# setarehc/diffusion-motion-inbetweening

Measured on NVIDIA H100. Metric: denoising steps/sec (B=64, L=196, D=263, 1000 steps), higher is better.
Workload: dtype bf16x3 (bf16 hi/lo operand split, fp32 accumulate: fp32-parity mode)

## Files before the change

diffusion-motion-inbetweening_b200/csrc/attention.cu:

```cuda
#include "common.cuh"
#include "gemm_epilogue.cuh"
#include "kernels.h"

namespace cmdi {

namespace {

constexpr int kHeadDim = 128;
constexpr int kQTile = 128;
constexpr int kKeyPad = kAttnKeyPad;
constexpr int kKeyBlocks = kKeyPad / 16;
constexpr int kQBlockBytes = kQTile * 128;
constexpr int kKVBlockBytes = kKeyPad * 128;
constexpr int kQPlane = 2 * kQBlockBytes;
constexpr int kKVPlane = 2 * kKVBlockBytes;
constexpr int kOffQHi = 0, kOffQLo = kQPlane;
constexpr int kOffKHi = 2 * kQPlane, kOffKLo = kOffKHi + kKVPlane;
constexpr int kOffVHi = kOffKLo + kKVPlane;
constexpr int kOffVLo = 0;
constexpr int kSmemTiles = kOffVHi + kKVPlane;
constexpr int kThreads = 256;
static_assert(kKVBlockBytes % 1024 == 0 && kKVPlane <= 2 * kQPlane, "operand tile layout");

struct __align__(8) AttnBarriers {
  uint64_t qkv_full, vlo_full;
};

__global__ void __launch_bounds__(kThreads, 1)
attention_kernel(const __grid_constant__ CUtensorMap map_q_hi, const __grid_constant__ CUtensorMap map_q_lo,
                 const __grid_constant__ CUtensorMap map_kv_hi, const __grid_constant__ CUtensorMap map_kv_lo, const AttnParams p) {
  extern __shared__ uint8_t smem_raw[];
  uint8_t* smem = reinterpret_cast<uint8_t*>((reinterpret_cast<uintptr_t>(smem_raw) + 1023) & ~uintptr_t(1023));
  AttnBarriers* bars = reinterpret_cast<AttnBarriers*>(smem + kSmemTiles);
  const int S = p.seq_len;
  const bool split = (p.nsplit == 3);
  const int half = blockIdx.x & 1;
  const int item = blockIdx.x >> 1;
  const int head = item % p.num_heads, seq = item / p.num_heads;
  if (half * kQTile >= S) return;
  const int warp_idx = threadIdx.x >> 5, lane = threadIdx.x & 31;
  const int wg = warp_idx >> 2, w = warp_idx & 3;
  const uint32_t sbase = smem_u32(smem);
  const int row0 = seq * S;
  const int kcol = p.num_heads * kHeadDim + head * kHeadDim, vcol = 2 * p.num_heads * kHeadDim + head * kHeadDim;
  const uint32_t planes = split ? 2 : 1;

  if (threadIdx.x == 0) {
    tma_prefetch_desc(&map_q_hi);
    tma_prefetch_desc(&map_kv_hi);
    mbar_init(&bars->qkv_full, 1);
    mbar_init(&bars->vlo_full, 1);
    fence_barrier_init();
    mbar_arrive_expect_tx(&bars->qkv_full, planes * (kQPlane + kKVPlane) + kKVPlane);
    for (int j = 0; j < 2; ++j) {
      tma_load_2d(smem + kOffQHi + j * kQBlockBytes, &map_q_hi, &bars->qkv_full, head * kHeadDim + j * 64, row0 + half * kQTile);
      tma_load_2d(smem + kOffKHi + j * kKVBlockBytes, &map_kv_hi, &bars->qkv_full, kcol + j * 64, row0);
      tma_load_2d(smem + kOffVHi + j * kKVBlockBytes, &map_kv_hi, &bars->qkv_full, vcol + j * 64, row0);
      if (split) {
        tma_load_2d(smem + kOffQLo + j * kQBlockBytes, &map_q_lo, &bars->qkv_full, head * kHeadDim + j * 64, row0 + half * kQTile);
        tma_load_2d(smem + kOffKLo + j * kKVBlockBytes, &map_kv_lo, &bars->qkv_full, kcol + j * 64, row0);
      }
    }
  }
  __syncthreads();

  float s[kKeyPad / 2];
  mbar_wait(&bars->qkv_full, 0);
  wgmma_fence_operands(s);
  wgmma_fence();
  {
    const int nterms = split ? 3 : 1;
#pragma unroll
    for (int term = 0; term < 3; ++term) {
      if (term >= nterms) break;
      const uint32_t qo = (split && term == 0) ? kOffQLo : kOffQHi;
      const uint32_t ko = (split && term == 1) ? kOffKLo : kOffKHi;
#pragma unroll
      for (int j = 0; j < 2; ++j) {
        const uint64_t da = make_desc_kmajor_sw128(sbase + qo + j * kQBlockBytes + wg * 64 * 128);
        const uint64_t db = make_desc_kmajor_sw128(sbase + ko + j * kKVBlockBytes);
#pragma unroll
        for (int kk = 0; kk < 4; ++kk)
          wgmma_m64n208k16_ss(s, desc_advance(da, kk * 32), desc_advance(db, kk * 32), (term | j | kk) ? 1u : 0u);
      }
    }
  }
  wgmma_commit();
  wgmma_wait<0>();
  wgmma_fence_operands(s);
  __syncthreads();
  if (split && threadIdx.x == 0) {
    mbar_arrive_expect_tx(&bars->vlo_full, kKVPlane);
    for (int j = 0; j < 2; ++j)
      tma_load_2d(smem + kOffVLo + j * kKVBlockBytes, &map_kv_lo, &bars->vlo_full, vcol + j * 64, row0);
  }

  const float c_scale = 0.08838834764831845f * 1.4426950408889634f;
  const int cq = 2 * (lane & 3);
  float mx0 = -INFINITY, mx1 = -INFINITY;
#pragma unroll
  for (int j = 0; j < kKeyPad / 8; ++j) {
    const bool ok0 = 8 * j + cq < S, ok1 = 8 * j + cq + 1 < S;
    if (!ok0) { s[4 * j] = -INFINITY; s[4 * j + 2] = -INFINITY; }
    if (!ok1) { s[4 * j + 1] = -INFINITY; s[4 * j + 3] = -INFINITY; }
    mx0 = fmaxf(mx0, fmaxf(s[4 * j], s[4 * j + 1]));
    mx1 = fmaxf(mx1, fmaxf(s[4 * j + 2], s[4 * j + 3]));
  }
#pragma unroll
  for (int o = 1; o <= 2; o <<= 1) {
    mx0 = fmaxf(mx0, __shfl_xor_sync(0xffffffffu, mx0, o));
    mx1 = fmaxf(mx1, __shfl_xor_sync(0xffffffffu, mx1, o));
  }
  const float mc0 = mx0 * c_scale, mc1 = mx1 * c_scale;
  float sum0 = 0.f, sum1 = 0.f;
  const bool trunc = p.trunc_split != 0;
  uint32_t ph[kKeyBlocks][4], pl[kKeyBlocks][4];
#pragma unroll
  for (int t = 0; t < kKeyBlocks; ++t) {
#pragma unroll
    for (int q = 0; q < 4; ++q) {
      const int i = 8 * t + 4 * (q >> 1) + 2 * (q & 1);
      const float mc = (q & 1) ? mc1 : mc0;
      const float p0 = fast_exp2(fmaf(s[i], c_scale, -mc));
      const float p1 = fast_exp2(fmaf(s[i + 1], c_scale, -mc));
      if (q & 1) sum1 += p0 + p1; else sum0 += p0 + p1;
      if (trunc) split_bf16x2_trunc(p0, p1, ph[t][q], pl[t][q]); else split_bf16x2(p0, p1, ph[t][q], pl[t][q]);
    }
  }
#pragma unroll
  for (int o = 1; o <= 2; o <<= 1) {
    sum0 += __shfl_xor_sync(0xffffffffu, sum0, o);
    sum1 += __shfl_xor_sync(0xffffffffu, sum1, o);
  }

  float o[kHeadDim / 2];
  const uint64_t dv_hi = make_desc_mnmajor_sw128(sbase + kOffVHi, kKVBlockBytes);
  wgmma_fence_operands(o);
  wgmma_fence();
  if (split) {
#pragma unroll
    for (int t = 0; t < kKeyBlocks; ++t) wgmma_m64n128k16_rs_tb(o, pl[t], desc_advance(dv_hi, t * 2048), t ? 1u : 0u);
  }
#pragma unroll
  for (int t = 0; t < kKeyBlocks; ++t) wgmma_m64n128k16_rs_tb(o, ph[t], desc_advance(dv_hi, t * 2048), (split || t) ? 1u : 0u);
  wgmma_commit();
  if (split) {
    mbar_wait(&bars->vlo_full, 0);
    const uint64_t dv_lo = make_desc_mnmajor_sw128(sbase + kOffVLo, kKVBlockBytes);
#pragma unroll
    for (int t = 0; t < kKeyBlocks; ++t) wgmma_m64n128k16_rs_tb(o, ph[t], desc_advance(dv_lo, t * 2048), 1u);
    wgmma_commit();
  }
  wgmma_wait<0>();
  wgmma_fence_operands(o);

  const float inv0 = 1.0f / sum0, inv1 = 1.0f / sum1;
  const int q0 = half * kQTile + wg * 64 + 16 * w + (lane >> 2);
#pragma unroll
  for (int g = 0; g < 2; ++g) {
    const int q = q0 + 8 * g;
    if (q >= S) continue;
    const float inv = g ? inv1 : inv0;
    const size_t off = (size_t)(row0 + q) * p.ld_out + head * kHeadDim + cq;
#pragma unroll
    for (int j = 0; j < kHeadDim / 8; ++j) {
      uint32_t hw, lw;
      if (trunc) split_bf16x2_trunc(o[4 * j + 2 * g] * inv, o[4 * j + 2 * g + 1] * inv, hw, lw);
      else split_bf16x2(o[4 * j + 2 * g] * inv, o[4 * j + 2 * g + 1] * inv, hw, lw);
      *reinterpret_cast<uint32_t*>(p.out_hi + off + 8 * j) = hw;
      if (p.nsplit_out == 3) *reinterpret_cast<uint32_t*>(p.out_lo + off + 8 * j) = lw;
    }
  }
}

}

cudaError_t configure_attention_kernel() {
  return cudaFuncSetAttribute(attention_kernel, cudaFuncAttributeMaxDynamicSharedMemorySize,
                              (int)(1024 + kSmemTiles + sizeof(AttnBarriers)));
}

cudaError_t launch_attention(const AttnMaps& m, const AttnParams& p, cudaStream_t stream) {
  if (p.seq_len > kKeyPad || p.seq_len < 1 || (p.nsplit != 1 && p.nsplit != 3)) {
    set_last_error("launch_attention: unsupported seq_len=%d nsplit=%d", p.seq_len, p.nsplit);
    return cudaErrorInvalidValue;
  }
  const int num_items = p.num_heads * p.num_seqs;
  const size_t smem = 1024 + kSmemTiles + sizeof(AttnBarriers);
  return launch_kernel(attention_kernel, dim3(2 * num_items), dim3(kThreads), smem, stream, *m.q_hi, *m.q_lo, *m.kv_hi, *m.kv_lo, p);
}

}
```

Before: 208.2.

## Make attention kernel persistent with per-operand barriers and next-item TMA prefetch

Converts the one-block-per-(seq,head,half) attention kernel into a persistent kernel with one block per SM looping over work items. Q, K-hi, K-lo, V-hi and V-lo get separate mbarriers with phase tracking, so the next item's operands can be loaded by TMA while the current item's softmax and PV run. V-lo now reuses the K-lo region instead of the Q region, which lets Q be prefetched early. The aim is to hide load latency and per-block launch/setup cost. The trade-offs are extra syncthreads, a cudaGetDevice/attribute query on every launch, and serialised item processing within each SM, since only one block fits per SM.

Result: no change. 210.0, median of 6 (+0.9%).

```diff
diff --git a/diffusion-motion-inbetweening_b200/csrc/attention.cu b/diffusion-motion-inbetweening_b200/csrc/attention.cu
--- a/diffusion-motion-inbetweening_b200/csrc/attention.cu
+++ b/diffusion-motion-inbetweening_b200/csrc/attention.cu
@@ -15,16 +15,46 @@
 constexpr int kQPlane = 2 * kQBlockBytes;
 constexpr int kKVPlane = 2 * kKVBlockBytes;
 constexpr int kOffQHi = 0, kOffQLo = kQPlane;
-constexpr int kOffKHi = 2 * kQPlane, kOffKLo = kOffKHi + kKVPlane;
+constexpr int kOffKHi = 2 * kQPlane;
+constexpr int kOffKLo = kOffKHi + kKVPlane, kOffVLo = kOffKLo;
 constexpr int kOffVHi = kOffKLo + kKVPlane;
-constexpr int kOffVLo = 0;
 constexpr int kSmemTiles = kOffVHi + kKVPlane;
 constexpr int kThreads = 256;
-static_assert(kKVBlockBytes % 1024 == 0 && kKVPlane <= 2 * kQPlane, "operand tile layout");
+static_assert(kKVBlockBytes % 1024 == 0, "operand tile layout");
 
 struct __align__(8) AttnBarriers {
-  uint64_t qkv_full, vlo_full;
+  uint64_t q_full, khi_full, klo_full, vhi_full, vlo_full;
 };
+
+struct AttnItem {
+  int row0, qrow, kcol, vcol, head;
+};
+
+__device__ __forceinline__ AttnItem attn_item(int it, int nhalves, const AttnParams& p) {
+  const int half = it % nhalves, hs = it / nhalves;
+  const int head = hs % p.num_heads, seq = hs / p.num_heads;
+  AttnItem r;
+  r.row0 = seq * p.seq_len;
+  r.qrow = r.row0 + half * kQTile;
+  r.head = head;
+  r.kcol = p.num_heads * kHeadDim + head * kHeadDim;
+  r.vcol = 2 * p.num_heads * kHeadDim + head * kHeadDim;
+  return r;
+}
+
+__device__ __forceinline__ void load_kv_plane(uint8_t* dst, const CUtensorMap* map, uint64_t* bar, int col, int row0) {
+  mbar_arrive_expect_tx(bar, kKVPlane);
+  for (int j = 0; j < 2; ++j) tma_load_2d(dst + j * kKVBlockBytes, map, bar, col + j * 64, row0);
+}
+
+__device__ __forceinline__ void load_q(uint8_t* smem, const CUtensorMap* map_hi, const CUtensorMap* map_lo, uint64_t* bar,
+                                       const AttnItem& t, bool split) {
+  mbar_arrive_expect_tx(bar, (split ? 2 : 1) * kQPlane);
+  for (int j = 0; j < 2; ++j) {
+    tma_load_2d(smem + kOffQHi + j * kQBlockBytes, map_hi, bar, t.head * kHeadDim + j * 64, t.qrow);
+    if (split) tma_load_2d(smem + kOffQLo + j * kQBlockBytes, map_lo, bar, t.head * kHeadDim + j * 64, t.qrow);
+  }
+}
 
 __global__ void __launch_bounds__(kThreads, 1)
 attention_kernel(const __grid_constant__ CUtensorMap map_q_hi, const __grid_constant__ CUtensorMap map_q_lo,
@@ -34,141 +64,153 @@
   AttnBarriers* bars = reinterpret_cast<AttnBarriers*>(smem + kSmemTiles);
   const int S = p.seq_len;
   const bool split = (p.nsplit == 3);
-  const int half = blockIdx.x & 1;
-  const int item = blockIdx.x >> 1;
-  const int head = item % p.num_heads, seq = item / p.num_heads;
-  if (half * kQTile >= S) return;
+  const int nhalves = (S + kQTile - 1) / kQTile;
+  const int num_items = nhalves * p.num_heads * p.num_seqs;
   const int warp_idx = threadIdx.x >> 5, lane = threadIdx.x & 31;
   const int wg = warp_idx >> 2, w = warp_idx & 3;
   const uint32_t sbase = smem_u32(smem);
-  const int row0 = seq * S;
-  const int kcol = p.num_heads * kHeadDim + head * kHeadDim, vcol = 2 * p.num_heads * kHeadDim + head * kHeadDim;
-  const uint32_t planes = split ? 2 : 1;
-
-  if (threadIdx.x == 0) {
+  const bool trunc = p.trunc_split != 0;
+  const int cq = 2 * (lane & 3);
+
+  if (threadIdx.x == 0 && (int)blockIdx.x < num_items) {
     tma_prefetch_desc(&map_q_hi);
     tma_prefetch_desc(&map_kv_hi);
-    mbar_init(&bars->qkv_full, 1);
+    mbar_init(&bars->q_full, 1);
+    mbar_init(&bars->khi_full, 1);
+    mbar_init(&bars->klo_full, 1);
+    mbar_init(&bars->vhi_full, 1);
     mbar_init(&bars->vlo_full, 1);
     fence_barrier_init();
-    mbar_arrive_expect_tx(&bars->qkv_full, planes * (kQPlane + kKVPlane) + kKVPlane);
-    for (int j = 0; j < 2; ++j) {
-      tma_load_2d(smem + kOffQHi + j * kQBlockBytes, &map_q_hi, &bars->qkv_full, head * kHeadDim + j * 64, row0 + half * kQTile);
-      tma_load_2d(smem + kOffKHi + j * kKVBlockBytes, &map_kv_hi, &bars->qkv_full, kcol + j * 64, row0);
-      tma_load_2d(smem + kOffVHi + j * kKVBlockBytes, &map_kv_hi, &bars->qkv_full, vcol + j * 64, row0);
-      if (split) {
-        tma_load_2d(smem + kOffQLo + j * kQBlockBytes, &map_q_lo, &bars->qkv_full, head * kHeadDim + j * 64, row0 + half * kQTile);
-        tma_load_2d(smem + kOffKLo + j * kKVBlockBytes, &map_kv_lo, &bars->qkv_full, kcol + j * 64, row0);
-      }
-    }
+    const AttnItem t = attn_item(blockIdx.x, nhalves, p);
+    load_q(smem, &map_q_hi, &map_q_lo, &bars->q_full, t, split);
+    load_kv_plane(smem + kOffKHi, &map_kv_hi, &bars->khi_full, t.kcol, t.row0);
+    if (split) load_kv_plane(smem + kOffKLo, &map_kv_lo, &bars->klo_full, t.kcol, t.row0);
+    load_kv_plane(smem + kOffVHi, &map_kv_hi, &bars->vhi_full, t.vcol, t.row0);
   }
   __syncthreads();
 
-  float s[kKeyPad / 2];
-  mbar_wait(&bars->qkv_full, 0);
-  wgmma_fence_operands(s);
-  wgmma_fence();
-  {
-    const int nterms = split ? 3 : 1;
-#pragma unroll
-    for (int term = 0; term < 3; ++term) {
-      if (term >= nterms) break;
-      const uint32_t qo = (split && term == 0) ? kOffQLo : kOffQHi;
-      const uint32_t ko = (split && term == 1) ? kOffKLo : kOffKHi;
-#pragma unroll
-      for (int j = 0; j < 2; ++j) {
-        const uint64_t da = make_desc_kmajor_sw128(sbase + qo + j * kQBlockBytes + wg * 64 * 128);
-        const uint64_t db = make_desc_kmajor_sw128(sbase + ko + j * kKVBlockBytes);
-#pragma unroll
-        for (int kk = 0; kk < 4; ++kk)
-          wgmma_m64n208k16_ss(s, desc_advance(da, kk * 32), desc_advance(db, kk * 32), (term | j | kk) ? 1u : 0u);
-      }
-    }
-  }
-  wgmma_commit();
-  wgmma_wait<0>();
-  wgmma_fence_operands(s);
-  __syncthreads();
-  if (split && threadIdx.x == 0) {
-    mbar_arrive_expect_tx(&bars->vlo_full, kKVPlane);
-    for (int j = 0; j < 2; ++j)
-      tma_load_2d(smem + kOffVLo + j * kKVBlockBytes, &map_kv_lo, &bars->vlo_full, vcol + j * 64, row0);
-  }
-
-  const float c_scale = 0.08838834764831845f * 1.4426950408889634f;
-  const int cq = 2 * (lane & 3);
-  float mx0 = -INFINITY, mx1 = -INFINITY;
-#pragma unroll
-  for (int j = 0; j < kKeyPad / 8; ++j) {
-    const bool ok0 = 8 * j + cq < S, ok1 = 8 * j + cq + 1 < S;
-    if (!ok0) { s[4 * j] = -INFINITY; s[4 * j + 2] = -INFINITY; }
-    if (!ok1) { s[4 * j + 1] = -INFINITY; s[4 * j + 3] = -INFINITY; }
-    mx0 = fmaxf(mx0, fmaxf(s[4 * j], s[4 * j + 1]));
-    mx1 = fmaxf(mx1, fmaxf(s[4 * j + 2], s[4 * j + 3]));
-  }
-#pragma unroll
-  for (int o = 1; o <= 2; o <<= 1) {
-    mx0 = fmaxf(mx0, __shfl_xor_sync(0xffffffffu, mx0, o));
-    mx1 = fmaxf(mx1, __shfl_xor_sync(0xffffffffu, mx1, o));
-  }
-  const float mc0 = mx0 * c_scale, mc1 = mx1 * c_scale;
-  float sum0 = 0.f, sum1 = 0.f;
-  const bool trunc = p.trunc_split != 0;
-  uint32_t ph[kKeyBlocks][4], pl[kKeyBlocks][4];
-#pragma unroll
-  for (int t = 0; t < kKeyBlocks; ++t) {
-#pragma unroll
-    for (int q = 0; q < 4; ++q) {
-      const int i = 8 * t + 4 * (q >> 1) + 2 * (q & 1);
-      const float mc = (q & 1) ? mc1 : mc0;
-      const float p0 = fast_exp2(fmaf(s[i], c_scale, -mc));
-      const float p1 = fast_exp2(fmaf(s[i + 1], c_scale, -mc));
-      if (q & 1) sum1 += p0 + p1; else sum0 += p0 + p1;
-      if (trunc) split_bf16x2_trunc(p0, p1, ph[t][q], pl[t][q]); else split_bf16x2(p0, p1, ph[t][q], pl[t][q]);
-    }
-  }
-#pragma unroll
-  for (int o = 1; o <= 2; o <<= 1) {
-    sum0 += __shfl_xor_sync(0xffffffffu, sum0, o);
-    sum1 += __shfl_xor_sync(0xffffffffu, sum1, o);
-  }
-
-  float o[kHeadDim / 2];
-  const uint64_t dv_hi = make_desc_mnmajor_sw128(sbase + kOffVHi, kKVBlockBytes);
-  wgmma_fence_operands(o);
-  wgmma_fence();
-  if (split) {
-#pragma unroll
-    for (int t = 0; t < kKeyBlocks; ++t) wgmma_m64n128k16_rs_tb(o, pl[t], desc_advance(dv_hi, t * 2048), t ? 1u : 0u);
-  }
-#pragma unroll
-  for (int t = 0; t < kKeyBlocks; ++t) wgmma_m64n128k16_rs_tb(o, ph[t], desc_advance(dv_hi, t * 2048), (split || t) ? 1u : 0u);
-  wgmma_commit();
-  if (split) {
-    mbar_wait(&bars->vlo_full, 0);
-    const uint64_t dv_lo = make_desc_mnmajor_sw128(sbase + kOffVLo, kKVBlockBytes);
-#pragma unroll
-    for (int t = 0; t < kKeyBlocks; ++t) wgmma_m64n128k16_rs_tb(o, ph[t], desc_advance(dv_lo, t * 2048), 1u);
+  uint32_t phase = 0;
+  for (int it = blockIdx.x; it < num_items; it += gridDim.x, phase ^= 1) {
+    const int next = it + (int)gridDim.x;
+
+    float s[kKeyPad / 2];
+    mbar_wait(&bars->q_full, phase);
+    mbar_wait(&bars->khi_full, phase);
+    wgmma_fence_operands(s);
+    wgmma_fence();
+    {
+      const int nterms = split ? 3 : 1;
+#pragma unroll
+      for (int term = 0; term < 3; ++term) {
+        if (term >= nterms) break;
+        if (term == 1) mbar_wait(&bars->klo_full, phase);
+        const uint32_t qo = (split && term == 0) ? kOffQLo : kOffQHi;
+        const uint32_t ko = (split && term == 1) ? kOffKLo : kOffKHi;
+#pragma unroll
+        for (int j = 0; j < 2; ++j) {
+          const uint64_t da = make_desc_kmajor_sw128(sbase + qo + j * kQBlockBytes + wg * 64 * 128);
+          const uint64_t db = make_desc_kmajor_sw128(sbase + ko + j * kKVBlockBytes);
+#pragma unroll
+          for (int kk = 0; kk < 4; ++kk)
+            wgmma_m64n208k16_ss(s, desc_advance(da, kk * 32), desc_advance(db, kk * 32), (term | j | kk) ? 1u : 0u);
+        }
+      }
+    }
     wgmma_commit();
-  }
-  wgmma_wait<0>();
-  wgmma_fence_operands(o);
-
-  const float inv0 = 1.0f / sum0, inv1 = 1.0f / sum1;
-  const int q0 = half * kQTile + wg * 64 + 16 * w + (lane >> 2);
-#pragma unroll
-  for (int g = 0; g < 2; ++g) {
-    const int q = q0 + 8 * g;
-    if (q >= S) continue;
-    const float inv = g ? inv1 : inv0;
-    const size_t off = (size_t)(row0 + q) * p.ld_out + head * kHeadDim + cq;
-#pragma unroll
-    for (int j = 0; j < kHeadDim / 8; ++j) {
-      uint32_t hw, lw;
-      if (trunc) split_bf16x2_trunc(o[4 * j + 2 * g] * inv, o[4 * j + 2 * g + 1] * inv, hw, lw);
-      else split_bf16x2(o[4 * j + 2 * g] * inv, o[4 * j + 2 * g + 1] * inv, hw, lw);
-      *reinterpret_cast<uint32_t*>(p.out_hi + off + 8 * j) = hw;
-      if (p.nsplit_out == 3) *reinterpret_cast<uint32_t*>(p.out_lo + off + 8 * j) = lw;
+    wgmma_wait<0>();
+    wgmma_fence_operands(s);
+    __syncthreads();
+    if (threadIdx.x == 0) {
+      const AttnItem t = attn_item(it, nhalves, p);
+      if (split) load_kv_plane(smem + kOffVLo, &map_kv_lo, &bars->vlo_full, t.vcol, t.row0);
+      if (next < num_items) {
+        const AttnItem u = attn_item(next, nhalves, p);
+        load_q(smem, &map_q_hi, &map_q_lo, &bars->q_full, u, split);
+        load_kv_plane(smem + kOffKHi, &map_kv_hi, &bars->khi_full, u.kcol, u.row0);
+      }
+    }
+
+    const float c_scale = 0.08838834764831845f * 1.4426950408889634f;
+    float mx0 = -INFINITY, mx1 = -INFINITY;
+#pragma unroll
+    for (int j = 0; j < kKeyPad / 8; ++j) {
+      const bool ok0 = 8 * j + cq < S, ok1 = 8 * j + cq + 1 < S;
+      if (!ok0) { s[4 * j] = -INFINITY; s[4 * j + 2] = -INFINITY; }
+      if (!ok1) { s[4 * j + 1] = -INFINITY; s[4 * j + 3] = -INFINITY; }
+      mx0 = fmaxf(mx0, fmaxf(s[4 * j], s[4 * j + 1]));
+      mx1 = fmaxf(mx1, fmaxf(s[4 * j + 2], s[4 * j + 3]));
+    }
+#pragma unroll
+    for (int o = 1; o <= 2; o <<= 1) {
+      mx0 = fmaxf(mx0, __shfl_xor_sync(0xffffffffu, mx0, o));
+      mx1 = fmaxf(mx1, __shfl_xor_sync(0xffffffffu, mx1, o));
+    }
+    const float mc0 = mx0 * c_scale, mc1 = mx1 * c_scale;
+    float sum0 = 0.f, sum1 = 0.f;
+    uint32_t ph[kKeyBlocks][4], pl[kKeyBlocks][4];
+#pragma unroll
+    for (int t = 0; t < kKeyBlocks; ++t) {
+#pragma unroll
+      for (int q = 0; q < 4; ++q) {
+        const int i = 8 * t + 4 * (q >> 1) + 2 * (q & 1);
+        const float mc = (q & 1) ? mc1 : mc0;
+        const float p0 = fast_exp2(fmaf(s[i], c_scale, -mc));
+        const float p1 = fast_exp2(fmaf(s[i + 1], c_scale, -mc));
+        if (q & 1) sum1 += p0 + p1; else sum0 += p0 + p1;
+        if (trunc) split_bf16x2_trunc(p0, p1, ph[t][q], pl[t][q]); else split_bf16x2(p0, p1, ph[t][q], pl[t][q]);
+      }
+    }
+#pragma unroll
+    for (int o = 1; o <= 2; o <<= 1) {
+      sum0 += __shfl_xor_sync(0xffffffffu, sum0, o);
+      sum1 += __shfl_xor_sync(0xffffffffu, sum1, o);
+    }
+
+    float o[kHeadDim / 2];
+    const uint64_t dv_hi = make_desc_mnmajor_sw128(sbase + kOffVHi, kKVBlockBytes);
+    mbar_wait(&bars->vhi_full, phase);
+    wgmma_fence_operands(o);
+    wgmma_fence();
+    if (split) {
+#pragma unroll
+      for (int t = 0; t < kKeyBlocks; ++t) wgmma_m64n128k16_rs_tb(o, pl[t], desc_advance(dv_hi, t * 2048), t ? 1u : 0u);
+    }
+#pragma unroll
+    for (int t = 0; t < kKeyBlocks; ++t) wgmma_m64n128k16_rs_tb(o, ph[t], desc_advance(dv_hi, t * 2048), (split || t) ? 1u : 0u);
+    wgmma_commit();
+    if (split) {
+      mbar_wait(&bars->vlo_full, phase);
+      const uint64_t dv_lo = make_desc_mnmajor_sw128(sbase + kOffVLo, kKVBlockBytes);
+#pragma unroll
+      for (int t = 0; t < kKeyBlocks; ++t) wgmma_m64n128k16_rs_tb(o, ph[t], desc_advance(dv_lo, t * 2048), 1u);
+      wgmma_commit();
+    }
+    wgmma_wait<0>();
+    wgmma_fence_operands(o);
+    __syncthreads();
+    if (threadIdx.x == 0 && next < num_items) {
+      const AttnItem u = attn_item(next, nhalves, p);
+      if (split) load_kv_plane(smem + kOffKLo, &map_kv_lo, &bars->klo_full, u.kcol, u.row0);
+      load_kv_plane(smem + kOffVHi, &map_kv_hi, &bars->vhi_full, u.vcol, u.row0);
+    }
+
+    const float inv0 = 1.0f / sum0, inv1 = 1.0f / sum1;
+    const AttnItem t = attn_item(it, nhalves, p);
+    const int q0 = (t.qrow - t.row0) + wg * 64 + 16 * w + (lane >> 2);
+#pragma unroll
+    for (int g = 0; g < 2; ++g) {
+      const int q = q0 + 8 * g;
+      if (q >= S) continue;
+      const float inv = g ? inv1 : inv0;
+      const size_t off = (size_t)(t.row0 + q) * p.ld_out + t.head * kHeadDim + cq;
+#pragma unroll
+      for (int j = 0; j < kHeadDim / 8; ++j) {
+        uint32_t hw, lw;
+        if (trunc) split_bf16x2_trunc(o[4 * j + 2 * g] * inv, o[4 * j + 2 * g + 1] * inv, hw, lw);
+        else split_bf16x2(o[4 * j + 2 * g] * inv, o[4 * j + 2 * g + 1] * inv, hw, lw);
+        *reinterpret_cast<uint32_t*>(p.out_hi + off + 8 * j) = hw;
+        if (p.nsplit_out == 3) *reinterpret_cast<uint32_t*>(p.out_lo + off + 8 * j) = lw;
+      }
     }
   }
 }
@@ -185,9 +227,14 @@
     set_last_error("launch_attention: unsupported seq_len=%d nsplit=%d", p.seq_len, p.nsplit);
     return cudaErrorInvalidValue;
   }
-  const int num_items = p.num_heads * p.num_seqs;
+  int dev = 0, num_sms = 0;
+  cudaError_t e = cudaGetDevice(&dev);
+  if (e == cudaSuccess) e = cudaDeviceGetAttribute(&num_sms, cudaDevAttrMultiProcessorCount, dev);
+  if (e != cudaSuccess) return e;
+  const int num_items = (p.seq_len + kQTile - 1) / kQTile * p.num_heads * p.num_seqs;
+  const int grid = num_items < num_sms ? num_items : num_sms;
   const size_t smem = 1024 + kSmemTiles + sizeof(AttnBarriers);
-  return launch_kernel(attention_kernel, dim3(2 * num_items), dim3(kThreads), smem, stream, *m.q_hi, *m.q_lo, *m.kv_hi, *m.kv_lo, p);
-}
-
-}
+  return launch_kernel(attention_kernel, dim3(grid), dim3(kThreads), smem, stream, *m.q_hi, *m.q_lo, *m.kv_hi, *m.kv_lo, p);
+}
+
+}
```
